# bobochow/adapt-image-models

Measured on AMD Instinct MI355X. Metric: clips/sec (8-frame 224^2 ViT-B/16 AIM fwd+bwd), higher is better.
Workload: dtype bf16; 1 GPU; BASELINE configs[1]: ViT-B/16 + AIM adapters, 8 frames 224^2, 64 clips/GPU, K400-shaped synthetic clips (400 random labels), fwd+bwd+AdamW; global_batch=64, frames=8, parallelism=dp1

## Files before the change

adapt-image-models_amd/backbone.py:

```python
import logging
import os
from collections import OrderedDict
from typing import Dict, List, Optional

import torch
from torch import nn

from . import ops
from .registry import BACKBONES

BF16, F32 = torch.bfloat16, torch.float32
_LOG = logging.getLogger("aim_amd")


def get_root_logger():
    return _LOG


class Adapter(nn.Module):

    def __init__(self, D_features: int, mlp_ratio: float = 0.25, skip_connect: bool = True):
        super().__init__()
        self.skip_connect = skip_connect
        hidden = int(D_features * mlp_ratio)
# ... 475 lines not shown
        return x2, None
    x1 = _empty((M, D), F32, dev)
    ops.gemm(ao, fz.Wo, ops.EPI_F32, x1, bias=fz.bo, resid=x, af=oml, vec=sv, bt=dms1, ntok=N)
    x2, xn, mean2, rstd2, hcat_pre, a_s = _mlp_adapter_forward(x1, fz, dms2, N, save)
    ctx = None
    if save:
        ctx = dict(x=x, mean1=mean1, rstd1=rstd1, qkv=qkv, probs=probs, ta=ta, t_pre=t_pre, t_h=t_h, lam=lam,
                   oml=oml, ao=ao, lse=lse, sin=sin, s_pre=s_pre, s_h=s_h, x1=x1, mean2=mean2, rstd2=rstd2, xn=xn,
                   hcat_pre=hcat_pre, a_s=a_s, dms1=dms1, dms2=dms2)
    return x2, ctx


def _mlp_adapter_forward(x1, fz: _Frozen, dms2, N, save: bool):
    dev = x1.device
    M, D = x1.shape
    r, H4 = fz.r, 4 * D
    xn = _empty((M, D), BF16, dev)
    mean2, rstd2 = _empty((M,), F32, dev), _empty((M,), F32, dev)
    ops.layernorm_fwd(x1, fz.g2, fz.b2, M, D, D, y_bf16=xn, mean=mean2, rstd=rstd2)
    frag = _AUX_FRAG and M >= 1024
    if frag:
        hcat_pre = ops.frag_buffer(M, H4 + r, dev) if save else None
    else:
        hcat_pre = _empty((M, H4 + r), BF16, dev) if (save or M < 1024) else None
    hcat = _empty((M, H4 + r), BF16, dev)
    ops.gemm(xn, fz.Wcat1, ops.EPI_ACT, hcat, bias=fz.bcat1, out2=hcat_pre, act=ops.ACT_QGELU, n_split=H4,
             act2=ops.ACT_GELU, at=dms2, ntok=N, aux_grad=_AUX_GRAD, aux_frag=frag and hcat_pre is not None)
    x2 = _empty((M, D), F32, dev)
    ops.gemm(hcat, fz.Wcat2, ops.EPI_F32, x2, bias=fz.bpr, resid=x1, vec=fz.b2row, ldv=0, bt=dms2, ntok=N)
    a_s = hcat[:, H4:] if save else None
    return x2, xn, mean2, rstd2, hcat_pre, a_s


def _mlp_adapter_backward(dyb, x_in, mean2, rstd2, xn, hcat_pre, a_s, dms2, fz: _Frozen, gm, N, fsum=None):
    dev = dyb.device
    M, D = dyb.shape
    r, H4 = fz.r, 4 * D
    big_later: list = []
    if _DETACH_BIG:
        big_later.append(lambda: ops.wgrad(dyb, a_s, gm["D_fc2.weight"], gm["D_fc2.bias"], at=dms2, ntok=N))
    else:
        ops.wgrad(dyb, a_s, gm["D_fc2.weight"], gm["D_fc2.bias"], at=dms2, ntok=N)
    dcat = _empty((M, H4 + r), BF16, dev)
    ops.gemm(dyb, fz.WcatT2, ops.EPI_DACT, dcat, aux=hcat_pre, act=ops.ACT_QGELU, n_split=H4, act2=ops.ACT_GELU,
             at=dms2, ntok=N, aux_grad=_AUX_GRAD, aux_frag=_AUX_FRAG and dyb.shape[0] >= 1024, reserve_cus=_DP_RESERVE)
    if _DETACH_BIG:
        big_later.append(lambda: ops.wgrad(dcat[:, H4:], xn, gm["D_fc1.weight"], gm["D_fc1.bias"]))
    else:
        ops.wgrad(dcat[:, H4:], xn, gm["D_fc1.weight"], gm["D_fc1.bias"])
    dxn = _empty((M, D), BF16, dev)
    ops.gemm(dcat, fz.WcatT1, ops.EPI_BF16, dxn, reserve_cus=_DP_RESERVE)
    dxb = _empty((M, D), BF16, dev)
    if fsum is not None:
        ops.layernorm_bwd_fsum(dxn, x_in, fz.g2, mean2, rstd2, dyb, dxb, fsum[0], fsum[1], M // N, N, D)
    else:
        ops.layernorm_bwd(dxn, x_in, fz.g2, mean2, rstd2, M, D, lddy=D, ldx=D, lddx=D, dres=dyb, dx_bf16=dxb)
    return dxb, big_later


def _adapter_bwd_small(dout_bf, ad: _AdapterW, a_in, pre, h, grads, rows, r, D, ar: _Arena, need_dx_bf16: bool, later: list):
    later.append(lambda: ops.wgrad(dout_bf, h, grads["D_fc2.weight"], grads["D_fc2.bias"]))
    dpre = ar.take((rows, r), BF16)
    ops.gemm(dout_bf, ad.W2T, ops.EPI_DACT, dpre, aux=pre, act=ops.ACT_GELU, aux_grad=_AUX_GRAD)
    later.append(lambda: ops.wgrad(dpre, a_in, grads["D_fc1.weight"], grads["D_fc1.bias"]))
    din = ar.take((rows, D), BF16 if need_dx_bf16 else F32)
    ops.gemm(dpre, ad.W1T, ops.EPI_BF16 if need_dx_bf16 else ops.EPI_F32, din)
    return din


def _block_backward(dyb, c, fz: _Frozen, adp: Dict[str, _AdapterW], grads, B, T, N, H, keep: Optional[list] = None):
    dev = dyb.device
    M, D = dyb.shape
    BT = B * T
    r, H4 = fz.r, 4 * D
    fpart = _empty((BT, ops.LN_FSUM_GROUPS, D), F32, dev) if _FSUM_IN_LN else None
    dx1b, big_later = _mlp_adapter_backward(dyb, c["x1"], c["mean2"], c["rstd2"], c["xn"], c["hcat_pre"], c["a_s"], c["dms2"],
                                            fz, grads["MLP_Adapter"], N, fsum=(c["dms1"], fpart) if _FSUM_IN_LN else None)
    later: list = big_later
    ar = _Arena(dev, 48 * BT * D + (1 << 16))
    with _Fork(dev, "bwd") as fork:
        dsv = ar.take((BT, D), F32)
        if _FSUM_IN_LN:
            ops.frame_sum(fpart, None, dsv, BT, ops.LN_FSUM_GROUPS, D)
        else:
            ops.frame_sum(dx1b, c["dms1"], dsv, BT, N, D)
        dsv_b = ar.take((BT, D), BF16)
        ops.cast_bf16(dsv, dsv_b)
        dsin = _adapter_bwd_small(dsv_b, adp["S_Adapter"], c["sin"], c["s_pre"], c["s_h"], grads["S_Adapter"], BT, r,
                                  D, ar, need_dx_bf16=False, later=later)
        dcrs = ar.take((BT, D), BF16)
        ops.scale_rows(dsin, c["lam"], y=dcrs)
        dvx = ar.take((BT, D), BF16)
        ops.gemm(dcrs, fz.WoT, ops.EPI_BF16, dvx)
        dxt = ar.take((BT, D), BF16)
        ops.gemm(dvx, fz.WqkvT[:, 2 * D:], ops.EPI_BF16, dxt)
        dta = _adapter_bwd_small(dxt, adp["T_Adapter"], c["ta"], c["t_pre"], c["t_h"], grads["T_Adapter"], BT, r, D,
                                 ar, need_dx_bf16=True, later=later)
        dot = ar.take((BT, D), BF16)
        ops.gemm(dta, fz.WoT, ops.EPI_BF16, dot)
        if _LATE_JOIN:
            dqkv_cls = ar.take((BT, 3 * D), BF16)
            ops.cls_attn_bwd(c["qkv"], c["probs"], dot, dqkv_cls, B, T, N, H, compact=True)
            dxl_cls = ar.take((BT, D), F32)
            ops.gemm(dqkv_cls, fz.WqkvT, ops.EPI_F32, dxl_cls)
    if keep is None:
        keep = []
        fork.run_detached(later, keep)
        _Fork.join_detached(dev)
    else:
        fork.run_detached(later, keep)
    dao = _empty((M, D), BF16, dev)
    ops.gemm(dx1b, fz.WoT, ops.EPI_BF16, dao, af=c["oml"], ntok=N, reserve_cus=_DP_RESERVE)
    dqkv = _empty((M, 3 * D), BF16, dev)
    delta = _empty((BT, H, N), F32, dev)
    ops.attn_bwd(c["qkv"], c["ao"], dao, c["lse"], delta, dqkv, BT, N, H)
    del dao
    if not _LATE_JOIN:
        fork.join()
        ops.cls_attn_bwd(c["qkv"], c["probs"], dot, dqkv, B, T, N, H)
    dxl = _empty((M, D), BF16, dev)
    ops.gemm(dqkv, fz.WqkvT, ops.EPI_BF16, dxl, reserve_cus=_DP_RESERVE)
    del dqkv
    if _LATE_JOIN:
        fork.join()
        ops.add_rows(dxl, N * D, dxl_cls)
    dxb = _empty((M, D), BF16, dev)
    ops.layernorm_bwd(dxl, c["x"], fz.g1, c["mean1"], c["rstd1"], M, D, lddy=D, ldx=D, lddx=D, dres=dx1b, dx_bf16=dxb)
    return dxb


class _BackboneFn(torch.autograd.Function):

    @staticmethod
    def forward(ctx, model: "ViT_CLIP", grad_enabled: bool, imgs: torch.Tensor, *params: torch.Tensor):
        L, H = model.layers, model.heads
        B, C, T, Hh, Ww = imgs.shape
        D, p = model.width, model.patch_size
        G = Hh // p
        N = G * G + 1
        BT, M = B * T, B * T * N
        dev = imgs.device
        temporal, lnp_w, lnp_b = params[0], params[1], params[2]
        need_grad = grad_enabled and any(ctx.needs_input_grad)
# ... 375 lines not shown
```

adapt-image-models_amd/csrc/wgrad.hip:

```cpp
#include "aim_common.h"
#include <stdlib.h>
#include "aim_kernels_internal.h"

namespace {

constexpr int MSTEP = 32;
constexpr int NST = 4;
constexpr int IMG = MSTEP * 128;
constexpr int OPER_BYTES = 4 * IMG;
constexpr int STAGE_BYTES = 2 * OPER_BYTES;
constexpr int TILE = 256;

__global__ __launch_bounds__(512) void wgrad_kernel(const bf16_t* __restrict__ G, int ldg, const bf16_t* __restrict__ A,
                                                    int lda, float* __restrict__ dW, int lddw, float* __restrict__ partial,
                                                    int M, int Nw, int Kw, int chunk, float* __restrict__ db,
                                                    float* __restrict__ bias_partial, const float* __restrict__ at, int ntok) {
    extern __shared__ __attribute__((aligned(16))) char smem_raw[];
    AIM_LDS char* smem = (AIM_LDS char*)smem_raw;
    AIM_LDS float* sAt = (AIM_LDS float*)(smem + NST * STAGE_BYTES);
    const int tiles_k = (Kw + TILE - 1) / TILE;
    const int tiles = ((Nw + TILE - 1) / TILE) * tiles_k;
    const int cidx = blockIdx.x / tiles, tix = blockIdx.x - cidx * tiles;
    const int tn = tix / tiles_k, tk = tix - tn * tiles_k;
    const int n0 = tn * TILE, k0 = tk * TILE;
    const int mbeg = cidx * chunk;
    const int mend = min(M, mbeg + chunk);
    if (mbeg >= mend) return;

    const int tid = threadIdx.x, lane = tid & 63;
    const int wave = __builtin_amdgcn_readfirstlane(tid >> 6);
    const int wn = wave >> 2, wk = wave & 3;
    const int frow = lane & 15, fq = lane >> 4;

    const bf16_t* Gb = G + (long long)mbeg * ldg + n0;
    const bf16_t* Ab = A + (long long)mbeg * lda + k0;
    const int rows = mend - mbeg;
    aim_rsrc_words rG = make_rsrc_words(Gb, ((long long)(rows - 1) * ldg + min(TILE, Nw - n0)) * 2);
    aim_rsrc_words rA = make_rsrc_words(Ab, ((long long)(rows - 1) * lda + min(TILE, Kw - k0)) * 2);

    const int srow = lane >> 3, schunk = (lane & 7) ^ srow;
    unsigned vg0[2], va0[2];
    AIM_LDS char* pdst[2];
#pragma unroll
    for (int j = 0; j < 2; ++j) {
        const int piece = wave * 2 + j;
        const int img = piece >> 2, rg = piece & 3;
        const int r = rg * 8 + srow;
        const int col = img * 64 + schunk * 8;
        vg0[j] = n0 + col < Nw ? (unsigned)((r * ldg + col) * 2) : AIM_OOB;
        va0[j] = k0 + col < Kw ? (unsigned)((r * lda + col) * 2) : AIM_OOB;
        pdst[j] = smem + img * IMG + rg * 1024;
    }
    const unsigned gstep = (unsigned)(MSTEP * ldg * 2), astep = (unsigned)(MSTEP * lda * 2);
    auto stage = [&](int buf, int ms) {
#pragma unroll
        for (int j = 0; j < 2; ++j) {
            stage_piece_asm(rG, pdst[j] + buf * STAGE_BYTES, vg0[j] + (unsigned)ms * gstep);
            stage_piece_asm(rA, pdst[j] + buf * STAGE_BYTES + OPER_BYTES, va0[j] + (unsigned)ms * astep);
        }
    };

    f32x4 acc[8][4];
#pragma unroll
    for (int i = 0; i < 8; ++i)
#pragma unroll
        for (int j = 0; j < 4; ++j) acc[i][j] = f32x4{0.f, 0.f, 0.f, 0.f};

    auto frag = [&](const AIM_LDS char* oper, int c0) -> bf16x8 {
// ... 36 lines not shown
            const bf16x8 v1 = lds_read8(img + swz_off(brow + 16, bcg & 7));
            float f0 = 1.0f, f1 = 1.0f;
            if (at) {
                f0 = sAt[btok0];
                f1 = sAt[btok1];
                btok0 += bstep; if (btok0 >= ntok) btok0 -= ntok;
                btok1 += bstep; if (btok1 >= ntok) btok1 -= ntok;
            }
#pragma unroll
            for (int e = 0; e < 8; ++e) bs[e] += f0 * (float)v0[e] + f1 * (float)v1[e];
        }
        bf16x8 gf[8], af[4];
#pragma unroll
        for (int j = 0; j < 4; ++j) af[j] = frag(sA, wk * 64 + j * 16);
#pragma unroll
        for (int i = 0; i < 8; ++i) gf[i] = frag(sG, wn * 128 + i * 16);
#pragma unroll
        for (int i = 0; i < 8; ++i)
#pragma unroll
            for (int j = 0; j < 4; ++j)
                acc[i][j] = __builtin_amdgcn_mfma_f32_16x16x32_bf16(af[j], gf[i], acc[i][j], 0, 0, 0);
    }
    asm volatile("s_waitcnt vmcnt(0)" ::: "memory");
    if (do_bias) {
        __syncthreads();
        AIM_LDS float* red = (AIM_LDS float*)smem;
#pragma unroll
        for (int e = 0; e < 8; ++e) red[brow * 256 + bcg * 8 + e] = bs[e];
        __syncthreads();
        if (tid < 256 && n0 + tid < Nw) {
            float v = 0.f;
#pragma unroll
            for (int r = 0; r < 16; ++r) v += red[r * 256 + tid];
            if (bias_partial) bias_partial[(long long)cidx * Nw + n0 + tid] = v;
            else db[n0 + tid] += v;
        }
    }
    float* slab = partial ? partial + (long long)cidx * Nw * Kw : nullptr;
#pragma unroll
    for (int i = 0; i < 8; ++i)
#pragma unroll
        for (int j = 0; j < 4; ++j) {
            const int n = n0 + wn * 128 + i * 16 + frow;
            const int k = k0 + wk * 64 + j * 16 + fq * 4;
            if (n >= Nw || k >= Kw) continue;
            if (slab) *(f32x4*)(slab + (long long)n * Kw + k) = acc[i][j];
            else
#pragma unroll
                for (int e = 0; e < 4; ++e) atomicAdd(dW + (long long)n * lddw + k + e, acc[i][j][e]);
        }
}

__global__ __launch_bounds__(256) void wgrad_finish_kernel(const float* __restrict__ partial, float* __restrict__ dW,
                                                           int lddw, int nchunks, int Nw, int Kw,
                                                           const float* __restrict__ bias_partial, float* __restrict__ db) {
    const long long total = (long long)Nw * Kw;
    const long long idx = ((long long)blockIdx.x * 256 + threadIdx.x) * 4;
    if (idx < total) {
        f32x4 acc = f32x4{0.f, 0.f, 0.f, 0.f};
        int c = 0;
        for (; c + 8 <= nchunks; c += 8) {
            f32x4 v[8];
#pragma unroll
            for (int j = 0; j < 8; ++j) v[j] = *(const f32x4*)(partial + (long long)(c + j) * total + idx);
#pragma unroll
            for (int j = 0; j < 8; ++j) acc += v[j];
        }
        for (; c < nchunks; ++c) acc += *(const f32x4*)(partial + (long long)c * total + idx);
        const int n = (int)(idx / Kw), k = (int)(idx - (long long)n * Kw);
        f32x4* o = (f32x4*)(dW + (long long)n * lddw + k);
        *o = *o + acc;
    }
    if (bias_partial) {
        const int n = blockIdx.x * 4 + (threadIdx.x >> 6), lane = threadIdx.x & 63;
        if (n < Nw) {
            float a = 0.f;
            for (int c = lane; c < nchunks; c += 64) a += bias_partial[(long long)c * Nw + n];
            a = wave_sum(a);
            if (lane == 0) db[n] += a;
        }
    }
}

__global__ __launch_bounds__(256) void wgrad_finish1_kernel(const float* __restrict__ partial, float* __restrict__ dW,
                                                            int lddw, int nchunks, int Nw, int Kw) {
    const long long idx = (long long)blockIdx.x * 256 + threadIdx.x;
    const long long total = (long long)Nw * Kw;
    if (idx >= total) return;
    float acc = 0.f;
    for (int c = 0; c < nchunks; ++c) acc += partial[(long long)c * total + idx];
    const int n = (int)(idx / Kw), k = (int)(idx - (long long)n * Kw);
    dW[(long long)n * lddw + k] += acc;
}

}

static int wgrad_chunks(int M, int tiles, int* chunk_out) {
    static const int target = [] { const char* e = getenv("AIM_WGRAD_WGS"); const int v = e ? atoi(e) : 256; return v > 0 ? v : 256; }();
    int nchunks = (target + tiles - 1) / tiles;
    const int maxchunks = (M + MSTEP - 1) / MSTEP;
    if (nchunks > maxchunks) nchunks = maxchunks;
    int chunk = (M + nchunks - 1) / nchunks;
    chunk = ((chunk + MSTEP - 1) / MSTEP) * MSTEP;
    if (chunk_out) *chunk_out = chunk;
    return (M + chunk - 1) / chunk;
}

extern "C" int64_t aim_wgrad_workspace_bytes(int M, int Nw, int Kw) {
    const int tiles = ((Nw + TILE - 1) / TILE) * ((Kw + TILE - 1) / TILE);
    const int nchunks = wgrad_chunks(M, tiles, nullptr);
    return nchunks > 1 ? (int64_t)nchunks * Nw * (Kw + 1) * 4 : 0;
}

extern "C" int aim_wgrad_bias_bf16(const aim_bf16* G, int ldg, const aim_bf16* A, int lda, float* dW, int lddw, float* db,
                                   const float* at, int ntok, int M, int Nw, int Kw, float* workspace, int64_t workspace_bytes,
                                   void* stream) {
    AIM_CHECK_ARG(M > 0 && Nw > 0 && Kw > 0 && (Nw % 8) == 0 && (Kw % 8) == 0, "wgrad: Nw/Kw must be positive multiples of 8 (Nw=%d Kw=%d)", Nw, Kw);
    AIM_CHECK_ARG((ldg % 8) == 0 && (lda % 8) == 0 && (lddw % 4) == 0, "wgrad: ldg/lda must be multiples of 8, lddw of 4");
    AIM_CHECK_ARG(G && A && dW, "wgrad: null pointer");
    AIM_CHECK_ARG(!at || (db && ntok > 0 && ntok <= 4096), "wgrad: row factors need db and 0 < ntok <= 4096");
    const int tiles = ((Nw + TILE - 1) / TILE) * ((Kw + TILE - 1) / TILE);
    int chunk = 0;
    const int nchunks = wgrad_chunks(M, tiles, &chunk);
    const int lds_bytes = NST * STAGE_BYTES + (at ? ((ntok * 4 + 15) & ~15) : 0);
    static bool attr_set = false;
    if (!attr_set) {
        (void)hipFuncSetAttribute((const void*)wgrad_kernel, hipFuncAttributeMaxDynamicSharedMemorySize, 160 * 1024);
        attr_set = true;
    }
    AIM_CHECK_ARG((long long)chunk * (ldg > lda ? ldg : lda) * 2 < 0x7fffffffLL, "wgrad: chunk too large");
    float* slab = (workspace && nchunks > 1 && workspace_bytes >= (int64_t)nchunks * Nw * (Kw + 1) * 4) ? workspace : nullptr;
    static const bool fuse_bias = [] { const char* e = getenv("AIM_WGRAD_FUSE_BIAS"); return !e || atoi(e) != 0; }();
    static const bool finish_v = [] { const char* e = getenv("AIM_WGRAD_FINISH_V"); return !e || atoi(e) != 0; }();
    float* bias_slab = (slab && db && fuse_bias) ? slab + (long long)nchunks * Nw * Kw : nullptr;
    if (db && nchunks > 1 && !bias_slab) {
        const int rc = aim_colsum_bf16(G, ldg, nullptr, at, ntok, db, M, Nw, nullptr, 0, stream);
        if (rc) return rc;
        db = nullptr;
    }
    hipLaunchKernelGGL(wgrad_kernel, dim3(tiles * nchunks), dim3(512), lds_bytes, (hipStream_t)stream,
                       (const bf16_t*)G, ldg, (const bf16_t*)A, lda, dW, lddw, slab, M, Nw, Kw, chunk, db, bias_slab, at, ntok);
    AIM_CHECK_LAUNCH("aim_wgrad_bf16");
    if (slab) {
        const long long total = (long long)Nw * Kw;
        unsigned fgrid = (unsigned)((total / 4 + 255) / 256);
        if (bias_slab && (unsigned)((Nw + 3) / 4) > fgrid) fgrid = (unsigned)((Nw + 3) / 4);
        if (finish_v || bias_slab)
            hipLaunchKernelGGL(wgrad_finish_kernel, dim3(fgrid), dim3(256), 0, (hipStream_t)stream,
                               slab, dW, lddw, nchunks, Nw, Kw, bias_slab, db);
        else
            hipLaunchKernelGGL(wgrad_finish1_kernel, dim3((unsigned)((total + 255) / 256)), dim3(256), 0, (hipStream_t)stream,
                               slab, dW, lddw, nchunks, Nw, Kw);
        AIM_CHECK_LAUNCH("aim_wgrad_bf16(finish)");
    }
    return 0;
}

extern "C" int aim_wgrad_bf16(const aim_bf16* G, int ldg, const aim_bf16* A, int lda, float* dW, int lddw, float* db,
                              int M, int Nw, int Kw, float* workspace, int64_t workspace_bytes, void* stream) {
    return aim_wgrad_bias_bf16(G, ldg, A, lda, dW, lddw, db, nullptr, 0, M, Nw, Kw, workspace, workspace_bytes, stream);
}
```

adapt-image-models_amd/lib.py:

```python
import ctypes
import os
from ctypes import POINTER, Structure, c_char_p, c_float, c_int, c_int32, c_int64, c_void_p

_HERE = os.path.dirname(os.path.abspath(__file__))
_LIB = None


class LibraryNotBuilt(RuntimeError):
    pass


def library_path() -> str:
    return os.environ.get("AIM_HIP_LIB") or os.path.join(_HERE, "libaim_hip.so")


class GemmArgs(Structure):
    _fields_ = [
        ("A", c_void_p), ("W", c_void_p), ("lda", c_int32), ("ldw", c_int32),
        ("strideA", c_int64), ("strideW", c_int64),
        ("M", c_int32), ("N", c_int32), ("K", c_int32),
        ("bias", c_void_p), ("resid", c_void_p), ("ldr", c_int32),
        ("af", c_void_p), ("at", c_void_p), ("vec", c_void_p), ("bt", c_void_p),
        ("ldv", c_int32), ("ntok", c_int32),
        ("aux", c_void_p), ("ldaux", c_int32),
        ("out", c_void_p), ("ldo", c_int32), ("out2", c_void_p), ("ldo2", c_int32),
        ("scale", c_float), ("act", c_int32), ("rs_bias_only", c_int32), ("n_split", c_int32), ("act2", c_int32),
        ("xrow", c_void_p), ("ldx", c_int32),
        ("reserve_cus", c_int32), ("probe", c_void_p), ("probe_cap", c_int32),
        ("wscale", c_void_p), ("aux_grad", c_int32), ("aux_frag", c_int32), ("row0", c_int32),
    ]


P = c_void_p
I = c_int
L = c_int64
F = c_float

SIGNATURES = {
    "aim_version": [],
    "aim_last_error": [],
    "aim_gemm_bf16": [POINTER(GemmArgs), I, I, P],
    "aim_gemm_fp8": [POINTER(GemmArgs), I, P],
    "aim_gemm_expsum_tiles": [I, I],
    "aim_wgrad_bf16": [P, I, P, I, P, I, P, I, I, I, P, L, P],
    "aim_wgrad_workspace_bytes": [I, I, I],
    "aim_wgrad_bias_bf16": [P, I, P, I, P, I, P, P, I, I, I, I, P, L, P],
    "aim_layernorm_fwd": [P, L, P, P, P, P, L, P, P, I, I, F, P],
    "aim_layernorm_fwd_fp8": [P, L, P, P, P, L, I, I, F, P],
    "aim_layernorm_fwd_x16": [P, L, P, P, P, P, P, L, I, I, F, P],
    "aim_layernorm_bwd": [P, I, L, P, L, P, P, P, P, I, P, P, L, P, P, I, I, P],
    "aim_layernorm_bwd_fsum": [P, L, P, L, P, P, P, P, P, L, P, P, I, I, I, I, P],
    "aim_attn_fwd": [P, P, P, I, I, I, P],
    "aim_attn_fwd_fp8": [P, P, P, I, I, I, P],
    "aim_attn_bwd": [P, P, P, P, P, P, I, I, I, P],
    "aim_cls_attn_fwd": [P, P, P, I, I, I, I, P],
    "aim_cls_attn_bwd": [P, P, P, P, I, I, I, I, I, P],
    "aim_tattn_fwd": [P, P, P, I, I, I, I, P],
    "aim_tattn_bwd": [P, P, P, P, I, I, I, I, P],
    "aim_add_bf16": [P, L, P, L, P, L, I, I, P],
    "aim_acc_bf16": [P, P, L, I, I, P],
    "aim_lambda_partials": [P, P, P, I, P],
    "aim_qk_cross": [P, P, I, P, I, I, I, F, P],
    "aim_lambda": [P, P, I, P, P, I, P, P, I, I, I, F, P],
    "aim_qk_border": [P, P, I, P, P, I, I, I, I, I, F, P],
    "aim_patchify": [P, I, P, P, P, I, I, I, I, I, I, P],
    "aim_patchify_blend": [P, I, P, P, P, I, I, I, I, I, I, P, I, F, F, I, I, I, I, P],
    "aim_embed_ln": [P, P, P, P, P, P, P, P, P, I, I, I, I, F, P],
    "aim_embed_bwd": [P, I, P, P, P, P, P, P, P, P, I, I, I, I, P, L, P],
    "aim_embed_bwd_workspace_bytes": [I, I, I, I],
    "aim_frame_sum": [P, I, P, P, I, I, I, P],
    "aim_colsum_bf16": [P, I, P, P, I, P, I, I, P, L, P],
    "aim_cast_bf16": [P, P, I, I, I, I, P],
    "aim_scale_rows": [P, P, P, P, I, I, P],
    "aim_add_rows_bf16": [P, L, P, I, I, P],
    "aim_adamw_flat": [P, P, P, P, L, F, F, F, F, F, I, F, P],
    "aim_head_fwd": [P, P, P, P, P, P, I, I, I, I, P],
    "aim_head_bwd": [P, P, P, P, P, P, P, I, I, I, I, P],
    "aim_ce_topk": [P, P, P, P, P, I, I, I, P],
    "aim_ce_soft": [P, P, P, P, P, P, I, I, P],
    "aim_cast_multi": [P, I, P],
    "aim_gemm_f32": [POINTER(GemmArgs), I, I, P],
    "aim_attn_fwd_f32": [P, P, I, I, I, P],
    "aim_cls_attn_fwd_f32": [P, L, P, I, I, I, P],
    "aim_lambda_f32": [P, I, P, P, I, P, P, I, I, I, F, P],
    "aim_patchify_f32": [P, I, P, P, P, I, I, I, I, I, I, P],
    "aim_patchify_blend_f32": [P, I, P, P, P, I, I, I, I, I, I, P, I, F, F, I, I, I, I, P],
    "aim_embed_ln_f32": [P, P, P, P, P, P, P, P, P, P, I, I, I, I, F, P],
    "aim_attn_bwd_f32_workspace_bytes": [I, I, I],
    "aim_attn_bwd_f32": [P, P, P, I, I, I, P, L, P],
    "aim_cls_attn_bwd_f32": [P, L, P, P, I, I, I, P],
    "aim_tattn_fwd_f32": [P, P, I, I, I, I, P],
    "aim_tattn_bwd_f32": [P, P, P, I, I, I, I, P],
    "aim_wgrad_f32_workspace_bytes": [I, I, I],
    "aim_wgrad_f32": [P, I, P, I, P, I, I, I, P, P, I, P, L, P],
    "aim_embed_nopre_fwd": [P, P, P, P, P, I, I, I, I, P],
    "aim_embed_nopre_bwd_workspace_bytes": [I, I, I, I],
    "aim_embed_nopre_bwd": [P, I, P, P, P, P, P, I, I, I, I, P, L, P],
    "aim_layernorm_gb_bwd_workspace_bytes": [I, I],
    "aim_layernorm_gb_bwd": [P, I, L, P, L, P, P, P, P, I, I, P, L, P],
}

ABI_VERSION = 8


def load_library():
    global _LIB
    if _LIB is not None:
        return _LIB
    path = library_path()
    if not os.path.exists(path):
        raise LibraryNotBuilt(
            f"{path} not found: build it with `python -c 'import __graft_entry__ as g; g.build()'` "
            f"(or `make -C adapt-image-models_amd/csrc`). There is no CPU fallback.")
    lib = ctypes.CDLL(path)
    for name, argtypes in SIGNATURES.items():
        fn = getattr(lib, name)
        fn.argtypes = argtypes
        fn.restype = c_char_p if name == "aim_last_error" else (c_int64 if name.endswith("_bytes") else c_int)
    if lib.aim_version() != ABI_VERSION:
        raise LibraryNotBuilt(f"{path}: ABI version {lib.aim_version()} != {ABI_VERSION}; rebuild")
    _LIB = lib
    return lib


def check(rc: int, what: str = ""):
    if rc != 0:
        msg = load_library().aim_last_error()
        raise RuntimeError(f"libaim_hip {what} failed (rc={rc}): {msg.decode() if msg else '?'}")
```

adapt-image-models_amd/ops.py:

```python
from ctypes import byref
from typing import Optional

import torch

from .lib import GemmArgs, check, load_library

EPI_BF16, EPI_ACT, EPI_DACT, EPI_F32, EPI_EXPSUM, EPI_ACT8, EPI_RES16 = 0, 1, 2, 3, 4, 5, 6
FP8 = torch.float8_e4m3fn
ACT_QGELU, ACT_GELU = 0, 1

BF16 = torch.bfloat16
F32 = torch.float32


_RAW_STREAM = getattr(torch._C, "_cuda_getCurrentRawStream", None)
_RAW_DEVICE = getattr(torch._C, "_cuda_getDevice", None)


def _stream() -> int:
    if _RAW_STREAM is not None:
        return _RAW_STREAM(_RAW_DEVICE())
    return torch.cuda.current_stream().cuda_stream


# ... 156 lines not shown
    q = (wf / scale[:, None]).clamp_(-448.0, 448.0)
    w8 = q.cpu().to(FP8).to(w.device)
    return w8.contiguous(), scale.contiguous()


def layernorm_fwd_fp8(x, gamma, beta, rows, D, ldx, y8, ldy=None, eps: float = 1e-5):
    _chk(x, F32, "x"); _chk(gamma, F32, "gamma"); _chk(beta, F32, "beta")
    if y8.element_size() != 1 or not y8.is_cuda:
        raise TypeError("y8: expected a GPU fp8 (1-byte) tensor")
    check(load_library().aim_layernorm_fwd_fp8(x.data_ptr(), ldx, gamma.data_ptr(), beta.data_ptr(), y8.data_ptr(),
                                               D if ldy is None else ldy, rows, D, eps, _stream()), "aim_layernorm_fwd_fp8")


def layernorm_fwd_x16(x, gamma, beta, rows, D, ldx, *, y_bf16=None, y_f32=None, y8=None, ldy=None, eps: float = 1e-5):
    _chk(x, BF16, "x"); _chk(gamma, F32, "gamma"); _chk(beta, F32, "beta"); _chk(y_bf16, BF16, "y_bf16"); _chk(y_f32, F32, "y_f32")
    if y8 is not None and (y8.element_size() != 1 or not y8.is_cuda):
        raise TypeError("y8: expected a GPU fp8 (1-byte) tensor")
    check(load_library().aim_layernorm_fwd_x16(x.data_ptr(), ldx, gamma.data_ptr(), beta.data_ptr(), _p(y_bf16), _p(y_f32), _p(y8),
                                               D if ldy is None else ldy, rows, D, eps, _stream()), "aim_layernorm_fwd_x16")


def attn_fwd_fp8(qkv, out8, BT, N, H, lse=None):
    _chk(qkv, BF16, "qkv"); _chk(lse, F32, "lse")
    if out8.element_size() != 1 or not out8.is_cuda:
        raise TypeError("out8: expected a GPU fp8 (1-byte) tensor")
    check(load_library().aim_attn_fwd_fp8(qkv.data_ptr(), out8.data_ptr(), _p(lse), BT, N, H, _stream()), "aim_attn_fwd_fp8")


def expsum_tiles(M: int, N: int) -> int:
    return load_library().aim_gemm_expsum_tiles(M, N)


def wgrad(g: torch.Tensor, a: torch.Tensor, dw: torch.Tensor, db: Optional[torch.Tensor] = None, at=None, ntok: int = 0):
    _chk(g, BF16, "g"); _chk(a, BF16, "a"); _chk(dw, F32, "dw"); _chk(db, F32, "db"); _chk(at, F32, "at")
    assert g.shape[0] == a.shape[0] and dw.shape == (g.shape[1], a.shape[1])
    lib = load_library()
    nbytes = lib.aim_wgrad_workspace_bytes(g.shape[0], g.shape[1], a.shape[1])
    ws = torch.empty(nbytes // 4, dtype=F32, device=g.device) if nbytes else None
    check(lib.aim_wgrad_bias_bf16(g.data_ptr(), g.stride(0), a.data_ptr(), a.stride(0), dw.data_ptr(), dw.stride(0), _p(db),
                                  _p(at), ntok, g.shape[0], g.shape[1], a.shape[1], _p(ws), nbytes, _stream()), "aim_wgrad_bias_bf16")


def layernorm_fwd(x, gamma, beta, rows, D, ldx, *, y_bf16=None, y_f32=None, ldy=None, mean=None, rstd=None,
                  eps: float = 1e-5):
    _chk(x, F32, "x"); _chk(gamma, F32, "gamma"); _chk(beta, F32, "beta")
    _chk(y_bf16, BF16, "y_bf16"); _chk(y_f32, F32, "y_f32"); _chk(mean, F32, "mean"); _chk(rstd, F32, "rstd")
    check(load_library().aim_layernorm_fwd(x.data_ptr(), ldx, gamma.data_ptr(), beta.data_ptr(), _p(y_bf16),
                                           _p(y_f32), D if ldy is None else ldy, _p(mean), _p(rstd), rows, D,
                                           eps, _stream()), "aim_layernorm_fwd")


def layernorm_bwd(dy, x, gamma, mean, rstd, rows, D, *, lddy, ldx, lddx, dres=None, dx=None, dx_bf16=None,
                  dgamma=None, dbeta=None):
    for n_, t_ in (("x", x), ("gamma", gamma), ("mean", mean), ("rstd", rstd),
                   ("dx", dx), ("dgamma", dgamma), ("dbeta", dbeta)):
        _chk(t_, F32, n_)
    _chk(dx_bf16, BF16, "dx_bf16")
    _chk(dy, dy.dtype if dy.dtype in (F32, BF16) else F32, "dy")
    if dres is not None:
        _chk(dres, dres.dtype if dres.dtype in (F32, BF16) else F32, "dres")
    check(load_library().aim_layernorm_bwd(dy.data_ptr(), int(dy.dtype == BF16), lddy, x.data_ptr(), ldx, gamma.data_ptr(),
                                           mean.data_ptr(), rstd.data_ptr(), _p(dres),
                                           int(dres is not None and dres.dtype == BF16), _p(dx), _p(dx_bf16), lddx,
                                           _p(dgamma), _p(dbeta), rows, D, _stream()), "aim_layernorm_bwd")


LN_FSUM_GROUPS = 13


def layernorm_bwd_fsum(dy, x, gamma, mean, rstd, dres, dx_bf16, w, partial, frames, ntok, D):
    _chk(dy, BF16, "dy"); _chk(dres, BF16, "dres"); _chk(dx_bf16, BF16, "dx_bf16")
    for n_, t_ in (("x", x), ("gamma", gamma), ("mean", mean), ("rstd", rstd), ("w", w), ("partial", partial)):
        _chk(t_, F32, n_)
# ... 405 lines not shown
```

include/aim_kernels.h:

```cpp
#ifndef AIM_KERNELS_H
#define AIM_KERNELS_H

#include <stdint.h>

#ifdef __cplusplus
extern "C" {
#endif

typedef uint16_t aim_bf16;

#define AIM_ABI_VERSION 8

int aim_version(void);
const char* aim_last_error(void);

enum {
    AIM_EPI_BF16 = 0,
    AIM_EPI_ACT = 1,
    AIM_EPI_DACT = 2,
    AIM_EPI_F32 = 3,
    AIM_EPI_EXPSUM = 4,
    AIM_EPI_ACT8 = 5,
    AIM_EPI_RES16 = 6
};
enum { AIM_ACT_QGELU = 0, AIM_ACT_GELU = 1 };

typedef struct aim_gemm_args {
    const aim_bf16* A;
    const aim_bf16* W;
    int32_t lda, ldw;
    int64_t strideA, strideW;
    int32_t M, N, K;
    const float* bias;
    const float* resid;
    int32_t ldr;
    const float* af;
    const float* at;
    const float* vec;
    const float* bt;
    int32_t ldv, ntok;
    const aim_bf16* aux;
    int32_t ldaux;
    void* out;  int32_t ldo;
    void* out2; int32_t ldo2;
    float scale;
    int32_t act;
    int32_t rs_bias_only;
    int32_t n_split, act2;
    const aim_bf16* xrow;
    int32_t ldx;
    int32_t reserve_cus;
    void* probe;
    int32_t probe_cap;
    const float* wscale;
    int32_t aux_grad;
    int32_t aux_frag;
    int32_t row0;
} aim_gemm_args;

int aim_gemm_bf16(const aim_gemm_args* args, int epilogue, int batch, void* stream);

int aim_gemm_fp8(const aim_gemm_args* args, int epilogue, void* stream);
int aim_gemm_expsum_tiles(int M, int N);

int aim_wgrad_bf16(const aim_bf16* G, int ldg, const aim_bf16* A, int lda, float* dW, int lddw,
                   float* db, int M, int Nw, int Kw,
                   float* workspace ,
                   int64_t workspace_bytes, void* stream);
int64_t aim_wgrad_workspace_bytes(int M, int Nw, int Kw);
int aim_wgrad_bias_bf16(const aim_bf16* G, int ldg, const aim_bf16* A, int lda, float* dW, int lddw, float* db,
                        const float* at, int ntok, int M, int Nw, int Kw, float* workspace, int64_t workspace_bytes, void* stream);

int aim_layernorm_fwd(const float* x, int64_t ldx, const float* gamma, const float* beta,
                      aim_bf16* y_bf16, float* y_f32, int64_t ldy, float* mean, float* rstd,
                      int rows, int D, float eps, void* stream);
int aim_layernorm_fwd_fp8(const float* x, int64_t ldx, const float* gamma, const float* beta, uint8_t* y_fp8,
                          int64_t ldy, int rows, int D, float eps, void* stream);
int aim_layernorm_fwd_x16(const aim_bf16* x, int64_t ldx, const float* gamma, const float* beta, aim_bf16* y_bf16,
                          float* y_f32, uint8_t* y_fp8, int64_t ldy, int rows, int D, float eps, void* stream);
int aim_layernorm_bwd(const void* dy, int dy_is_bf16 , int64_t lddy,
                      const float* x, int64_t ldx, const float* gamma,
                      const float* mean, const float* rstd, const void* dres, int dres_is_bf16, float* dx,
                      aim_bf16* dx_bf16, int64_t lddx, float* dgamma, float* dbeta,
                      int rows, int D, void* stream);
int aim_layernorm_bwd_fsum(const aim_bf16* dy, int64_t lddy, const float* x, int64_t ldx, const float* gamma,
                           const float* mean, const float* rstd, const aim_bf16* dres, aim_bf16* dx_bf16, int64_t lddx,
                           const float* w, float* fsum_partial, int groups, int frames, int ntok, int D, void* stream);

int aim_attn_fwd(const aim_bf16* qkv, aim_bf16* out, float* lse, int BT, int N, int H, void* stream);
int aim_attn_fwd_fp8(const aim_bf16* qkv, uint8_t* out_fp8, float* lse, int BT, int N, int H, void* stream);
int aim_attn_bwd(const aim_bf16* qkv, const aim_bf16* out, const aim_bf16* dout, const float* lse,
                 float* delta , aim_bf16* dqkv, int BT, int N, int H,
                 void* stream);

int aim_cls_attn_fwd(const aim_bf16* qkv, aim_bf16* out_cls, float* probs, int B, int T, int N, int H,
                     void* stream);
int aim_cls_attn_bwd(const aim_bf16* qkv, const float* probs, const aim_bf16* dout_cls, aim_bf16* dqkv, int compact,
                     int B, int T, int N, int H, void* stream);

int aim_tattn_fwd(const aim_bf16* qkv, aim_bf16* out, float* probs, int B, int T, int N, int H, void* stream);
int aim_tattn_bwd(const aim_bf16* qkv, const float* probs, const aim_bf16* dout, aim_bf16* dqkv, int B, int T, int N, int H,
                  void* stream);
int aim_add_bf16(const aim_bf16* a, int64_t lda, const aim_bf16* b, int64_t ldb, aim_bf16* out, int64_t ldo, int R, int C,
                 void* stream);
// ... 91 lines not shown
```

Before: 1272 clips/s.

## Batch per-block adapter weight-gradient GEMMs into one grouped launch

Result: no change. 1282 clips/s, median of 6 (+0.8%).

```diff
diff --git a/adapt-image-models_amd/backbone.py b/adapt-image-models_amd/backbone.py
--- a/adapt-image-models_amd/backbone.py
+++ b/adapt-image-models_amd/backbone.py
@@ -531,20 +531,31 @@
     return x2, xn, mean2, rstd2, hcat_pre, a_s
 
 
+class _WgradJob:
+    __slots__ = ("args",)
+
+    def __init__(self, g, a, dw, db=None, at=None, ntok: int = 0):
+        self.args = (g, a, dw, db, at, ntok)
+
+    def __call__(self):
+        g, a, dw, db, at, ntok = self.args
+        ops.wgrad(g, a, dw, db, at=at, ntok=ntok)
+
+
 def _mlp_adapter_backward(dyb, x_in, mean2, rstd2, xn, hcat_pre, a_s, dms2, fz: _Frozen, gm, N, fsum=None):
     dev = dyb.device
     M, D = dyb.shape
     r, H4 = fz.r, 4 * D
     big_later: list = []
     if _DETACH_BIG:
-        big_later.append(lambda: ops.wgrad(dyb, a_s, gm["D_fc2.weight"], gm["D_fc2.bias"], at=dms2, ntok=N))
+        big_later.append(_WgradJob(dyb, a_s, gm["D_fc2.weight"], gm["D_fc2.bias"], dms2, N))
     else:
         ops.wgrad(dyb, a_s, gm["D_fc2.weight"], gm["D_fc2.bias"], at=dms2, ntok=N)
     dcat = _empty((M, H4 + r), BF16, dev)
     ops.gemm(dyb, fz.WcatT2, ops.EPI_DACT, dcat, aux=hcat_pre, act=ops.ACT_QGELU, n_split=H4, act2=ops.ACT_GELU,
              at=dms2, ntok=N, aux_grad=_AUX_GRAD, aux_frag=_AUX_FRAG and dyb.shape[0] >= 1024, reserve_cus=_DP_RESERVE)
     if _DETACH_BIG:
-        big_later.append(lambda: ops.wgrad(dcat[:, H4:], xn, gm["D_fc1.weight"], gm["D_fc1.bias"]))
+        big_later.append(_WgradJob(dcat[:, H4:], xn, gm["D_fc1.weight"], gm["D_fc1.bias"]))
     else:
         ops.wgrad(dcat[:, H4:], xn, gm["D_fc1.weight"], gm["D_fc1.bias"])
     dxn = _empty((M, D), BF16, dev)
@@ -558,10 +569,10 @@
 
 
 def _adapter_bwd_small(dout_bf, ad: _AdapterW, a_in, pre, h, grads, rows, r, D, ar: _Arena, need_dx_bf16: bool, later: list):
-    later.append(lambda: ops.wgrad(dout_bf, h, grads["D_fc2.weight"], grads["D_fc2.bias"]))
+    later.append(_WgradJob(dout_bf, h, grads["D_fc2.weight"], grads["D_fc2.bias"]))
     dpre = ar.take((rows, r), BF16)
     ops.gemm(dout_bf, ad.W2T, ops.EPI_DACT, dpre, aux=pre, act=ops.ACT_GELU, aux_grad=_AUX_GRAD)
-    later.append(lambda: ops.wgrad(dpre, a_in, grads["D_fc1.weight"], grads["D_fc1.bias"]))
+    later.append(_WgradJob(dpre, a_in, grads["D_fc1.weight"], grads["D_fc1.bias"]))
     din = ar.take((rows, D), BF16 if need_dx_bf16 else F32)
     ops.gemm(dpre, ad.W1T, ops.EPI_BF16 if need_dx_bf16 else ops.EPI_F32, din)
     return din
@@ -602,12 +613,13 @@
             ops.cls_attn_bwd(c["qkv"], c["probs"], dot, dqkv_cls, B, T, N, H, compact=True)
             dxl_cls = ar.take((BT, D), F32)
             ops.gemm(dqkv_cls, fz.WqkvT, ops.EPI_F32, dxl_cls)
+    group = [lambda: ops.wgrad_group([j.args for j in later])]
     if keep is None:
         keep = []
-        fork.run_detached(later, keep)
+        fork.run_detached(group, keep)
         _Fork.join_detached(dev)
     else:
-        fork.run_detached(later, keep)
+        fork.run_detached(group, keep)
     dao = _empty((M, D), BF16, dev)
     ops.gemm(dx1b, fz.WoT, ops.EPI_BF16, dao, af=c["oml"], ntok=N, reserve_cus=_DP_RESERVE)
     dqkv = _empty((M, 3 * D), BF16, dev)
diff --git a/adapt-image-models_amd/csrc/wgrad.hip b/adapt-image-models_amd/csrc/wgrad.hip
--- a/adapt-image-models_amd/csrc/wgrad.hip
+++ b/adapt-image-models_amd/csrc/wgrad.hip
@@ -10,21 +10,52 @@
 constexpr int OPER_BYTES = 4 * IMG;
 constexpr int STAGE_BYTES = 2 * OPER_BYTES;
 constexpr int TILE = 256;
-
-__global__ __launch_bounds__(512) void wgrad_kernel(const bf16_t* __restrict__ G, int ldg, const bf16_t* __restrict__ A,
-                                                    int lda, float* __restrict__ dW, int lddw, float* __restrict__ partial,
-                                                    int M, int Nw, int Kw, int chunk, float* __restrict__ db,
-                                                    float* __restrict__ bias_partial, const float* __restrict__ at, int ntok) {
+constexpr int WG_SMALL_M = 2048;
+
+struct WgProb {
+    const bf16_t* G;
+    const bf16_t* A;
+    float* dW;
+    float* db;
+    const float* at;
+    float* slab;
+    float* bias_slab;
+    int ldg, lda, lddw, ntok, M, Nw, Kw;
+    int chunk, nchunks;
+    int blk0, nblk;
+    int xcd;
+};
+struct WgTable {
+    WgProb p[AIM_WGRAD_GROUP_MAX];
+    int n;
+};
+
+__device__ __forceinline__ int wg_find(const WgTable& T, int b) {
+    int pi = 0;
+#pragma unroll
+    for (int i = 1; i < AIM_WGRAD_GROUP_MAX; ++i)
+        if (i < T.n && b >= T.p[i].blk0) pi = i;
+    return pi;
+}
+
+__global__ __launch_bounds__(512) void wgrad_group_kernel(const WgTable T) {
     extern __shared__ __attribute__((aligned(16))) char smem_raw[];
     AIM_LDS char* smem = (AIM_LDS char*)smem_raw;
     AIM_LDS float* sAt = (AIM_LDS float*)(smem + NST * STAGE_BYTES);
+    const WgProb& P = T.p[wg_find(T, blockIdx.x)];
+    const int Nw = P.Nw, Kw = P.Kw, ldg = P.ldg, lda = P.lda, ntok = P.ntok;
+    const float* at = P.at;
+    float* db = P.db;
     const int tiles_k = (Kw + TILE - 1) / TILE;
     const int tiles = ((Nw + TILE - 1) / TILE) * tiles_k;
-    const int cidx = blockIdx.x / tiles, tix = blockIdx.x - cidx * tiles;
+    const int b = blockIdx.x - P.blk0;
+    const int w = P.nchunks > 1 && P.xcd ? (b & 7) * (P.nblk >> 3) + (b >> 3) : b;
+    if (w >= tiles * P.nchunks) return;
+    const int cidx = w / tiles, tix = w - cidx * tiles;
     const int tn = tix / tiles_k, tk = tix - tn * tiles_k;
     const int n0 = tn * TILE, k0 = tk * TILE;
-    const int mbeg = cidx * chunk;
-    const int mend = min(M, mbeg + chunk);
+    const int mbeg = cidx * P.chunk;
+    const int mend = min(P.M, mbeg + P.chunk);
     if (mbeg >= mend) return;
 
     const int tid = threadIdx.x, lane = tid & 63;
@@ -32,8 +63,8 @@
     const int wn = wave >> 2, wk = wave & 3;
     const int frow = lane & 15, fq = lane >> 4;
 
-    const bf16_t* Gb = G + (long long)mbeg * ldg + n0;
-    const bf16_t* Ab = A + (long long)mbeg * lda + k0;
+    const bf16_t* Gb = P.G + (long long)mbeg * ldg + n0;
+    const bf16_t* Ab = P.A + (long long)mbeg * lda + k0;
     const int rows = mend - mbeg;
     aim_rsrc_words rG = make_rsrc_words(Gb, ((long long)(rows - 1) * ldg + min(TILE, Nw - n0)) * 2);
     aim_rsrc_words rA = make_rsrc_words(Ab, ((long long)(rows - 1) * lda + min(TILE, Kw - k0)) * 2);
@@ -136,11 +167,14 @@
             float v = 0.f;
 #pragma unroll
             for (int r = 0; r < 16; ++r) v += red[r * 256 + tid];
-            if (bias_partial) bias_partial[(long long)cidx * Nw + n0 + tid] = v;
+            if (P.bias_slab) P.bias_slab[(long long)cidx * Nw + n0 + tid] = v;
             else db[n0 + tid] += v;
         }
     }
-    float* slab = partial ? partial + (long long)cidx * Nw * Kw : nullptr;
+    float* slab = P.slab ? P.slab + (long long)cidx * Nw * Kw : nullptr;
+    float* dW = P.dW;
+    const int lddw = P.lddw;
+    const bool single = P.nchunks == 1;
 #pragma unroll
     for (int i = 0; i < 8; ++i)
 #pragma unroll
@@ -149,17 +183,22 @@
             const int k = k0 + wk * 64 + j * 16 + fq * 4;
             if (n >= Nw || k >= Kw) continue;
             if (slab) *(f32x4*)(slab + (long long)n * Kw + k) = acc[i][j];
-            else
+            else if (single) {
+                f32x4* o = (f32x4*)(dW + (long long)n * lddw + k);
+                *o = *o + acc[i][j];
+            } else
 #pragma unroll
                 for (int e = 0; e < 4; ++e) atomicAdd(dW + (long long)n * lddw + k + e, acc[i][j][e]);
         }
 }
 
-__global__ __launch_bounds__(256) void wgrad_finish_kernel(const float* __restrict__ partial, float* __restrict__ dW,
-                                                           int lddw, int nchunks, int Nw, int Kw,
-                                                           const float* __restrict__ bias_partial, float* __restrict__ db) {
+__global__ __launch_bounds__(256) void wgrad_finish_kernel(const WgTable T) {
+    const WgProb& P = T.p[wg_find(T, blockIdx.x)];
+    const int b = blockIdx.x - P.blk0;
+    const int Nw = P.Nw, Kw = P.Kw, nchunks = P.nchunks;
+    const float* partial = P.slab;
     const long long total = (long long)Nw * Kw;
-    const long long idx = ((long long)blockIdx.x * 256 + threadIdx.x) * 4;
+    const long long idx = ((long long)b * 256 + threadIdx.x) * 4;
     if (idx < total) {
         f32x4 acc = f32x4{0.f, 0.f, 0.f, 0.f};
         int c = 0;
@@ -172,16 +211,16 @@
         }
         for (; c < nchunks; ++c) acc += *(const f32x4*)(partial + (long long)c * total + idx);
         const int n = (int)(idx / Kw), k = (int)(idx - (long long)n * Kw);
-        f32x4* o = (f32x4*)(dW + (long long)n * lddw + k);
+        f32x4* o = (f32x4*)(P.dW + (long long)n * P.lddw + k);
         *o = *o + acc;
     }
-    if (bias_partial) {
-        const int n = blockIdx.x * 4 + (threadIdx.x >> 6), lane = threadIdx.x & 63;
+    if (P.bias_slab) {
+        const int n = b * 4 + (threadIdx.x >> 6), lane = threadIdx.x & 63;
         if (n < Nw) {
             float a = 0.f;
-            for (int c = lane; c < nchunks; c += 64) a += bias_partial[(long long)c * Nw + n];
+            for (int c = lane; c < nchunks; c += 64) a += P.bias_slab[(long long)c * Nw + n];
             a = wave_sum(a);
-            if (lane == 0) db[n] += a;
+            if (lane == 0) P.db[n] += a;
         }
     }
 }
@@ -199,8 +238,12 @@
 
 }
 
-static int wgrad_chunks(int M, int tiles, int* chunk_out) {
+static int wgrad_target() {
     static const int target = [] { const char* e = getenv("AIM_WGRAD_WGS"); const int v = e ? atoi(e) : 256; return v > 0 ? v : 256; }();
+    return target;
+}
+
+static int wgrad_chunks(int M, int tiles, int target, int* chunk_out) {
     int nchunks = (target + tiles - 1) / tiles;
     const int maxchunks = (M + MSTEP - 1) / MSTEP;
     if (nchunks > maxchunks) nchunks = maxchunks;
@@ -210,9 +253,23 @@
     return (M + chunk - 1) / chunk;
 }
 
+static bool wgrad_xcd() {
+    static const bool on = [] { const char* e = getenv("AIM_WGRAD_XCD"); return !e || atoi(e) != 0; }();
+    return on;
+}
+
+static inline int wgrad_tiles(int Nw, int Kw) { return ((Nw + TILE - 1) / TILE) * ((Kw + TILE - 1) / TILE); }
+
+static void wgrad_set_lds_attr() {
+    static bool attr_set = false;
+    if (!attr_set) {
+        (void)hipFuncSetAttribute((const void*)wgrad_group_kernel, hipFuncAttributeMaxDynamicSharedMemorySize, 160 * 1024);
+        attr_set = true;
+    }
+}
+
 extern "C" int64_t aim_wgrad_workspace_bytes(int M, int Nw, int Kw) {
-    const int tiles = ((Nw + TILE - 1) / TILE) * ((Kw + TILE - 1) / TILE);
-    const int nchunks = wgrad_chunks(M, tiles, nullptr);
+    const int nchunks = wgrad_chunks(M, wgrad_tiles(Nw, Kw), wgrad_target(), nullptr);
     return nchunks > 1 ? (int64_t)nchunks * Nw * (Kw + 1) * 4 : 0;
 }
 
@@ -223,15 +280,11 @@
     AIM_CHECK_ARG((ldg % 8) == 0 && (lda % 8) == 0 && (lddw % 4) == 0, "wgrad: ldg/lda must be multiples of 8, lddw of 4");
     AIM_CHECK_ARG(G && A && dW, "wgrad: null pointer");
     AIM_CHECK_ARG(!at || (db && ntok > 0 && ntok <= 4096), "wgrad: row factors need db and 0 < ntok <= 4096");
-    const int tiles = ((Nw + TILE - 1) / TILE) * ((Kw + TILE - 1) / TILE);
+    const int tiles = wgrad_tiles(Nw, Kw);
     int chunk = 0;
-    const int nchunks = wgrad_chunks(M, tiles, &chunk);
+    const int nchunks = wgrad_chunks(M, tiles, wgrad_target(), &chunk);
     const int lds_bytes = NST * STAGE_BYTES + (at ? ((ntok * 4 + 15) & ~15) : 0);
-    static bool attr_set = false;
-    if (!attr_set) {
-        (void)hipFuncSetAttribute((const void*)wgrad_kernel, hipFuncAttributeMaxDynamicSharedMemorySize, 160 * 1024);
-        attr_set = true;
-    }
+    wgrad_set_lds_attr();
     AIM_CHECK_ARG((long long)chunk * (ldg > lda ? ldg : lda) * 2 < 0x7fffffffLL, "wgrad: chunk too large");
     float* slab = (workspace && nchunks > 1 && workspace_bytes >= (int64_t)nchunks * Nw * (Kw + 1) * 4) ? workspace : nullptr;
     static const bool fuse_bias = [] { const char* e = getenv("AIM_WGRAD_FUSE_BIAS"); return !e || atoi(e) != 0; }();
@@ -242,17 +295,24 @@
         if (rc) return rc;
         db = nullptr;
     }
-    hipLaunchKernelGGL(wgrad_kernel, dim3(tiles * nchunks), dim3(512), lds_bytes, (hipStream_t)stream,
-                       (const bf16_t*)G, ldg, (const bf16_t*)A, lda, dW, lddw, slab, M, Nw, Kw, chunk, db, bias_slab, at, ntok);
+    WgTable T = {};
+    T.n = 1;
+    WgProb& p = T.p[0];
+    p.G = (const bf16_t*)G; p.A = (const bf16_t*)A; p.dW = dW; p.db = db; p.at = db ? at : nullptr;
+    p.slab = slab; p.bias_slab = bias_slab;
+    p.ldg = ldg; p.lda = lda; p.lddw = lddw; p.ntok = ntok; p.M = M; p.Nw = Nw; p.Kw = Kw;
+    p.chunk = chunk; p.nchunks = nchunks; p.xcd = wgrad_xcd();
+    p.blk0 = 0; p.nblk = nchunks > 1 ? (tiles * nchunks + 7) / 8 * 8 : tiles;
+    hipLaunchKernelGGL(wgrad_group_kernel, dim3(p.nblk), dim3(512), lds_bytes, (hipStream_t)stream, T);
     AIM_CHECK_LAUNCH("aim_wgrad_bf16");
     if (slab) {
         const long long total = (long long)Nw * Kw;
         unsigned fgrid = (unsigned)((total / 4 + 255) / 256);
         if (bias_slab && (unsigned)((Nw + 3) / 4) > fgrid) fgrid = (unsigned)((Nw + 3) / 4);
-        if (finish_v || bias_slab)
-            hipLaunchKernelGGL(wgrad_finish_kernel, dim3(fgrid), dim3(256), 0, (hipStream_t)stream,
-                               slab, dW, lddw, nchunks, Nw, Kw, bias_slab, db);
-        else
+        if (finish_v || bias_slab) {
+            p.nblk = (int)fgrid;
+            hipLaunchKernelGGL(wgrad_finish_kernel, dim3(fgrid), dim3(256), 0, (hipStream_t)stream, T);
+        } else
             hipLaunchKernelGGL(wgrad_finish1_kernel, dim3((unsigned)((total + 255) / 256)), dim3(256), 0, (hipStream_t)stream,
                                slab, dW, lddw, nchunks, Nw, Kw);
         AIM_CHECK_LAUNCH("aim_wgrad_bf16(finish)");
@@ -264,3 +324,93 @@
                               int M, int Nw, int Kw, float* workspace, int64_t workspace_bytes, void* stream) {
     return aim_wgrad_bias_bf16(G, ldg, A, lda, dW, lddw, db, nullptr, 0, M, Nw, Kw, workspace, workspace_bytes, stream);
 }
+
+static int64_t wgrad_group_plan(const aim_wgrad_problem* in, int n, WgTable* compute, WgTable* finish, float* workspace) {
+    int nsplit = 0, small_blocks = 0;
+    for (int i = 0; i < n; ++i) {
+        if (in[i].M > WG_SMALL_M) ++nsplit;
+        else small_blocks += wgrad_tiles(in[i].Nw, in[i].Kw);
+    }
+    const int target = nsplit ? max(wgrad_target() - small_blocks, nsplit) / nsplit : 0;
+    *compute = WgTable{};
+    *finish = WgTable{};
+    int64_t ws = 0;
+    int blk = 0, fblk = 0;
+    for (int pass = 0; pass < 2; ++pass)
+        for (int i = 0; i < n; ++i) {
+            const aim_wgrad_problem& q = in[i];
+            const bool split = q.M > WG_SMALL_M;
+            if (split != (pass == 1)) continue;
+            const int tiles = wgrad_tiles(q.Nw, q.Kw);
+            WgProb& p = compute->p[compute->n++];
+            p.G = (const bf16_t*)q.G; p.A = (const bf16_t*)q.A; p.dW = q.dW; p.db = q.db; p.at = q.db ? q.at : nullptr;
+            p.ldg = q.ldg; p.lda = q.lda; p.lddw = q.lddw; p.ntok = q.ntok; p.M = q.M; p.Nw = q.Nw; p.Kw = q.Kw;
+            p.blk0 = blk;
+            p.xcd = wgrad_xcd();
+            if (!split) {
+                p.chunk = q.M; p.nchunks = 1; p.nblk = tiles;
+                blk += tiles;
+                continue;
+            }
+            blk = (blk + 7) / 8 * 8;
+            p.blk0 = blk;
+            p.nchunks = wgrad_chunks(q.M, tiles, max(target / tiles, 1) * tiles, &p.chunk);
+            p.nblk = (tiles * p.nchunks + 7) / 8 * 8;
+            blk += p.nblk;
+            const int64_t wbytes = (int64_t)p.nchunks * q.Nw * q.Kw * 4;
+            if (workspace) {
+                p.slab = workspace + ws / 4;
+                p.bias_slab = q.db ? p.slab + (long long)p.nchunks * q.Nw * q.Kw : nullptr;
+            }
+            ws += wbytes + (q.db ? (int64_t)p.nchunks * q.Nw * 4 : 0);
+            WgProb& f = finish->p[finish->n++];
+            f = p;
+            f.blk0 = fblk;
+            const long long total = (long long)q.Nw * q.Kw;
+            f.nblk = (int)((total / 4 + 255) / 256);
+            if (q.db && (q.Nw + 3) / 4 > f.nblk) f.nblk = (q.Nw + 3) / 4;
+            fblk += f.nblk;
+        }
+    return ws;
+}
+
+extern "C" int64_t aim_wgrad_group_workspace_bytes(const aim_wgrad_problem* probs, int n) {
+    if (!probs || n < 1 || n > AIM_WGRAD_GROUP_MAX) return 0;
+    WgTable c, f;
+    return wgrad_group_plan(probs, n, &c, &f, nullptr);
+}
+
+extern "C" int aim_wgrad_group_bf16(const aim_wgrad_problem* probs, int n, float* workspace, int64_t workspace_bytes,
+                                    void* stream) {
+    AIM_CHECK_ARG(probs && n >= 1 && n <= AIM_WGRAD_GROUP_MAX, "wgrad_group: 1 <= n <= %d problems (n=%d)", AIM_WGRAD_GROUP_MAX, n);
+    int at_bytes = 0;
+    for (int i = 0; i < n; ++i) {
+        const aim_wgrad_problem& q = probs[i];
+        AIM_CHECK_ARG(q.M > 0 && q.Nw > 0 && q.Kw > 0 && (q.Nw % 8) == 0 && (q.Kw % 8) == 0,
+                      "wgrad_group[%d]: M > 0, Nw/Kw positive multiples of 8 (M=%d Nw=%d Kw=%d)", i, q.M, q.Nw, q.Kw);
+        AIM_CHECK_ARG((q.ldg % 8) == 0 && (q.lda % 8) == 0 && (q.lddw % 4) == 0 && q.ldg >= q.Nw && q.lda >= q.Kw && q.lddw >= q.Kw,
+                      "wgrad_group[%d]: ldg/lda must be multiples of 8 and lddw of 4, each at least its row width", i);
+        AIM_CHECK_ARG(q.G && q.A && q.dW && ((uintptr_t)q.dW % 16) == 0, "wgrad_group[%d]: null pointer or dW not 16-byte aligned", i);
+        AIM_CHECK_ARG(!q.at || (q.db && q.ntok > 0 && q.ntok <= 4096), "wgrad_group[%d]: row factors need db and 0 < ntok <= 4096", i);
+        if (q.at && q.db) at_bytes = max(at_bytes, (q.ntok * 4 + 15) & ~15);
+    }
+    WgTable T, F;
+    const int64_t need = wgrad_group_plan(probs, n, &T, &F, workspace);
+    for (int i = 0; i < T.n; ++i)
+        AIM_CHECK_ARG((long long)T.p[i].chunk * (T.p[i].ldg > T.p[i].lda ? T.p[i].ldg : T.p[i].lda) * 2 < 0x7fffffffLL,
+                      "wgrad_group: chunk too large");
+    AIM_CHECK_ARG(need == 0 || (workspace && workspace_bytes >= need),
+                  "wgrad_group: workspace of %lld bytes needed (aim_wgrad_group_workspace_bytes), %lld given",
+                  (long long)need, (long long)workspace_bytes);
+    wgrad_set_lds_attr();
+    const WgProb& last = T.p[T.n - 1];
+    hipLaunchKernelGGL(wgrad_group_kernel, dim3(last.blk0 + last.nblk), dim3(512), NST * STAGE_BYTES + at_bytes,
+                       (hipStream_t)stream, T);
+    AIM_CHECK_LAUNCH("aim_wgrad_group_bf16");
+    if (F.n) {
+        const WgProb& fl = F.p[F.n - 1];
+        hipLaunchKernelGGL(wgrad_finish_kernel, dim3(fl.blk0 + fl.nblk), dim3(256), 0, (hipStream_t)stream, F);
+        AIM_CHECK_LAUNCH("aim_wgrad_group_bf16(finish)");
+    }
+    return 0;
+}
diff --git a/adapt-image-models_amd/lib.py b/adapt-image-models_amd/lib.py
--- a/adapt-image-models_amd/lib.py
+++ b/adapt-image-models_amd/lib.py
@@ -12,6 +12,17 @@
 
 def library_path() -> str:
     return os.environ.get("AIM_HIP_LIB") or os.path.join(_HERE, "libaim_hip.so")
+
+
+class WgradProblem(Structure):
+    _fields_ = [
+        ("G", c_void_p), ("A", c_void_p), ("dW", c_void_p), ("db", c_void_p), ("at", c_void_p),
+        ("ldg", c_int32), ("lda", c_int32), ("lddw", c_int32), ("ntok", c_int32),
+        ("M", c_int32), ("Nw", c_int32), ("Kw", c_int32),
+    ]
+
+
+WGRAD_GROUP_MAX = 6
 
 
 class GemmArgs(Structure):
@@ -45,6 +56,8 @@
     "aim_wgrad_bf16": [P, I, P, I, P, I, P, I, I, I, P, L, P],
     "aim_wgrad_workspace_bytes": [I, I, I],
     "aim_wgrad_bias_bf16": [P, I, P, I, P, I, P, P, I, I, I, I, P, L, P],
+    "aim_wgrad_group_workspace_bytes": [P, I],
+    "aim_wgrad_group_bf16": [P, I, P, L, P],
     "aim_layernorm_fwd": [P, L, P, P, P, P, L, P, P, I, I, F, P],
     "aim_layernorm_fwd_fp8": [P, L, P, P, P, L, I, I, F, P],
     "aim_layernorm_fwd_x16": [P, L, P, P, P, P, P, L, I, I, F, P],
@@ -100,7 +113,7 @@
     "aim_layernorm_gb_bwd": [P, I, L, P, L, P, P, P, P, I, I, P, L, P],
 }
 
-ABI_VERSION = 8
+ABI_VERSION = 9
 
 
 def load_library():
diff --git a/adapt-image-models_amd/ops.py b/adapt-image-models_amd/ops.py
--- a/adapt-image-models_amd/ops.py
+++ b/adapt-image-models_amd/ops.py
@@ -212,13 +212,27 @@
 
 
 def wgrad(g: torch.Tensor, a: torch.Tensor, dw: torch.Tensor, db: Optional[torch.Tensor] = None, at=None, ntok: int = 0):
-    _chk(g, BF16, "g"); _chk(a, BF16, "a"); _chk(dw, F32, "dw"); _chk(db, F32, "db"); _chk(at, F32, "at")
-    assert g.shape[0] == a.shape[0] and dw.shape == (g.shape[1], a.shape[1])
-    lib = load_library()
-    nbytes = lib.aim_wgrad_workspace_bytes(g.shape[0], g.shape[1], a.shape[1])
-    ws = torch.empty(nbytes // 4, dtype=F32, device=g.device) if nbytes else None
-    check(lib.aim_wgrad_bias_bf16(g.data_ptr(), g.stride(0), a.data_ptr(), a.stride(0), dw.data_ptr(), dw.stride(0), _p(db),
-                                  _p(at), ntok, g.shape[0], g.shape[1], a.shape[1], _p(ws), nbytes, _stream()), "aim_wgrad_bias_bf16")
+    wgrad_group([(g, a, dw, db, at, ntok)])
+
+
+def wgrad_group(problems):
+    from ctypes import addressof
+    from .lib import WGRAD_GROUP_MAX, WgradProblem
+    if not 1 <= len(problems) <= WGRAD_GROUP_MAX:
+        raise ValueError(f"wgrad_group: 1 to {WGRAD_GROUP_MAX} problems, got {len(problems)}")
+    table = (WgradProblem * len(problems))()
+    dev = problems[0][0].device
+    for p, (g, a, dw, db, at, ntok) in zip(table, problems):
+        _chk(g, BF16, "g"); _chk(a, BF16, "a"); _chk(dw, F32, "dw"); _chk(db, F32, "db"); _chk(at, F32, "at")
+        assert g.shape[0] == a.shape[0] and dw.shape == (g.shape[1], a.shape[1])
+        p.G, p.A, p.dW, p.db, p.at = g.data_ptr(), a.data_ptr(), dw.data_ptr(), _p(db), _p(at)
+        p.ldg, p.lda, p.lddw, p.ntok = g.stride(0), a.stride(0), dw.stride(0), ntok
+        p.M, p.Nw, p.Kw = g.shape[0], g.shape[1], a.shape[1]
+    lib = load_library()
+    ptr = addressof(table)
+    nbytes = lib.aim_wgrad_group_workspace_bytes(ptr, len(problems))
+    ws = torch.empty(nbytes // 4, dtype=F32, device=dev) if nbytes else None
+    check(lib.aim_wgrad_group_bf16(ptr, len(problems), _p(ws), nbytes, _stream()), "aim_wgrad_group_bf16")
 
 
 def layernorm_fwd(x, gamma, beta, rows, D, ldx, *, y_bf16=None, y_f32=None, ldy=None, mean=None, rstd=None,
diff --git a/include/aim_kernels.h b/include/aim_kernels.h
--- a/include/aim_kernels.h
+++ b/include/aim_kernels.h
@@ -9,7 +9,7 @@
 
 typedef uint16_t aim_bf16;
 
-#define AIM_ABI_VERSION 8
+#define AIM_ABI_VERSION 9
 
 int aim_version(void);
 const char* aim_last_error(void);
@@ -70,6 +70,17 @@
 int64_t aim_wgrad_workspace_bytes(int M, int Nw, int Kw);
 int aim_wgrad_bias_bf16(const aim_bf16* G, int ldg, const aim_bf16* A, int lda, float* dW, int lddw, float* db,
                         const float* at, int ntok, int M, int Nw, int Kw, float* workspace, int64_t workspace_bytes, void* stream);
+#define AIM_WGRAD_GROUP_MAX 6
+typedef struct aim_wgrad_problem {
+    const aim_bf16* G;
+    const aim_bf16* A;
+    float* dW;
+    float* db;
+    const float* at;
+    int32_t ldg, lda, lddw, ntok, M, Nw, Kw;
+} aim_wgrad_problem;
+int64_t aim_wgrad_group_workspace_bytes(const aim_wgrad_problem* probs, int n);
+int aim_wgrad_group_bf16(const aim_wgrad_problem* probs, int n, float* workspace, int64_t workspace_bytes, void* stream);
 
 int aim_layernorm_fwd(const float* x, int64_t ldx, const float* gamma, const float* beta,
                       aim_bf16* y_bf16, float* y_f32, int64_t ldy, float* mean, float* rstd,
```
